# rossng/oxmpl

Measured on AMD Instinct MI355X. Metric: RRT iterations/sec (batched problems), R^3 10k-node tree, 64-sphere field, higher is better.
Workload: dtype f64

## Files before the change

### oxmpl_amd/csrc/oxhip_api.hip

```cpp
#include "../../include/oxmpl_hip.h"

#include <algorithm>
#include <chrono>
#include <cmath>
#include <cstdio>
#include <cstring>
#include <limits>
#include <string>
#include <vector>

#include "oxhip_host.hpp"
#include "oxhip_internal.hpp"
#include "rrt_device.hpp"

using namespace oxhip;

#include <mutex>
#include <utility>
namespace {
std::mutex g_stream_mu;
std::vector<std::pair<int, hipStream_t>> g_stream_pool;
constexpr size_t kStreamPoolMax = 32;
}
namespace oxhip {
// ... 325 lines not shown
    chk(b->goal_r.alloc(P));
    if (!space_of(b).no_body && e == hipSuccess) {
        if (upload(b->se3_body, std::vector<double>(4 * (size_t)kSe3MaxBody, 0.0), b->stream) != OXHIP_OK) e = hipErrorOutOfMemory;
        b->se3.body = b->se3_body.p;
        b->se3.n_body = 1;
    }
    if (e != hipSuccess) return alloc_failed(e);
    dp.tree = b->tree.p; dp.parent = b->parent.p; dp.skip = b->skip.p; dp.state = b->state.p;
    dp.tree_b = b->tree_b.p; dp.parent_b = b->parent_b.p;
    dp.cost = b->cost.p; dp.nb_idx = b->nb_idx.p; dp.nb_dist = b->nb_dist.p;
    dp.wire_chk = b->wire_chk.p; dp.wired = b->wired.p; dp.nbr_cnt = b->nbr_cnt.p; dp.nbr_off = b->nbr_off.p;
    dp.nbr_take = b->nbr_take.p; dp.nbr_total = b->nbr_total.p; dp.d_near = b->d_near.p; dp.pool = b->pool.p;
    dp.chunks = b->chunks.p; dp.chunk_cursor = b->chunk_cursor.p;
    dp.goal_c = b->goal_c.p; dp.goal_thr = b->goal_thr.p; dp.goal_r = b->goal_r.p;
    return OXHIP_OK;
}

static int32_t alloc_cells(oxhip_rrt_batch* b) {
    DevParams& dp = b->dp;
    const uint32_t P = b->cfg.n_problems, dim = b->cfg.dim, cap = dp.cap;
    dp.cell_level_max = cells_level_max(dim, cap);
    dp.cell_blocks = cells_head_blocks(dim, cap) + cap / 7u + 64u;
    uint32_t split = b->cfg.frozen_split;
    if (split == 0) { split = (3072u + P - 1u) / P; if (split > 8u) split = 8u; if (split < 1u) split = 1u; }
    dp.cells_split = split;
    dp.sph_grid_G = sphere_grid_side(dim);
    const size_t grid_cells = dim == 2 ? (size_t)dp.sph_grid_G * dp.sph_grid_G : (size_t)dp.sph_grid_G * dp.sph_grid_G * dp.sph_grid_G;
    size_t off = 0;
    auto carve = [&](size_t bytes) { const size_t at = off; off = (off + bytes + 255u) & ~(size_t)255u; return at; };
    const size_t o_meta = carve((size_t)P * sizeof(CellMeta)), o_acc = carve((size_t)P * sizeof(CellAcc));
    const size_t zero_bytes = off;
    const size_t o_pos = carve((size_t)P * 64 * sizeof(uint64_t)), o_grid = carve(grid_cells * sizeof(uint64_t));
    const size_t o_grid2 = carve(b->star_wired ? grid_cells * sizeof(uint64_t) : 0);
    const size_t o_flat = carve((size_t)P * 4096 * 4 * sizeof(float)), o_xyz = carve((size_t)P * cap * 4 * sizeof(double));
    const size_t o_blk = carve((size_t)P * dp.cell_blocks * sizeof(CellBlock));
    hipError_t e = b->cell_arena.alloc(off);
    if (e == hipSuccess) e = hipMemset(b->cell_arena.p, 0, zero_bytes);
    if (e != hipSuccess) return alloc_failed(e);
    uint8_t* base = b->cell_arena.p;
    b->cell_meta_p = reinterpret_cast<CellMeta*>(base + o_meta);
    b->sph_grid_p = reinterpret_cast<uint64_t*>(base + o_grid);
    if (b->star_wired) b->star_grid_p = reinterpret_cast<uint64_t*>(base + o_grid2);
    dp.cell_blk = reinterpret_cast<CellBlock*>(base + o_blk); dp.cell_flat = reinterpret_cast<float*>(base + o_flat);
    dp.cell_xyz = reinterpret_cast<double*>(base + o_xyz); dp.cell_meta = b->cell_meta_p;
    dp.cell_acc = reinterpret_cast<CellAcc*>(base + o_acc); dp.cell_part_pos = reinterpret_cast<uint64_t*>(base + o_pos);
    dp.sph_grid = b->sph_grid_p;
    return OXHIP_OK;
}

static int32_t alloc_shadow(oxhip_rrt_batch* b) {
    const size_t P = b->cfg.n_problems;
    hipError_t e = b->tree32.alloc(P * b->cfg.dim * b->dp.cap);
    if (e == hipSuccess) e = b->shadow_state.alloc(P * 2);
    if (e == hipSuccess) e = hipMemset(b->shadow_state.p, 0, P * 2 * sizeof(uint32_t));
    if (e != hipSuccess) return alloc_failed(e);
    b->dp.tree32 = b->tree32.p;
    b->dp.shadow_state = b->shadow_state.p;
    return OXHIP_OK;
}

template <typename Launch>
static int32_t op_batch(int32_t device, const double* a, const double* b, const double* t, uint32_t n, double* out,
                        size_t w_a, size_t w_b, size_t w_out, bool b_uploaded, bool t_uploaded, Launch launch) {
    if (n == 0) return OXHIP_OK;
    OX_TRY(select_device(device));
    TmpStream ts;
    OX_TRY(ts.acquire(device));
    DevBuf<double> da, db, dt, dout;
// ... 1012 lines not shown
```

### oxmpl_amd/csrc/rrt_cells.hip

```cpp
#include "oxhip_internal.hpp"
#include "rrt_device.hpp"
#include "rrt_resident_common.hpp"
#include "lane_query_common.hpp"
#include "lane_sampler.hpp"

namespace oxhip {

#ifndef OXHIP_CELLS_BRUTE
#define OXHIP_CELLS_BRUTE 512
#endif
constexpr uint32_t kBruteMax = OXHIP_CELLS_BRUTE;
constexpr uint32_t kFlatCap = 4096;
static_assert(kBruteMax <= kFlatCap, "the flat list holds the small trees");
constexpr int kCellsWaves = 4;
constexpr uint32_t kSelfSkipMax = 4;
constexpr uint32_t kMaxSplit = 64;
constexpr int kMaxShell = 6;
#ifndef OXHIP_CELLS_NB
#define OXHIP_CELLS_NB 4
#endif
#ifndef OXHIP_ABLATE
#define OXHIP_ABLATE 0
#endif
#ifndef OXHIP_CELLS_WT_UNROLL
#define OXHIP_CELLS_WT_UNROLL 4
#endif
#ifndef OXHIP_CELLS_NB_FROZEN
#define OXHIP_CELLS_NB_FROZEN 3
#endif
#ifndef OXHIP_CELLS_FILL_X2
#define OXHIP_CELLS_FILL_X2 7ull
#endif
#ifndef OXHIP_CELLS_TAIL
#define OXHIP_CELLS_TAIL 64
#endif

typedef float cfloat4 __attribute__((ext_vector_type(4)));
typedef uint32_t cuint4 __attribute__((ext_vector_type(4)));
typedef double cdouble4 __attribute__((ext_vector_type(4)));
// ... 21 lines not shown
template <int DIM>
struct CellsShared {
    double obs[DIM + 2][64];
    CellsWaveLds<DIM> w[kCellsWaves];
};

__host__ __device__ __forceinline__ uint32_t cells_G(uint32_t level) {
    const uint32_t t[15] = {1u, 2u, 2u, 3u, 4u, 6u, 8u, 11u, 16u, 23u, 32u, 45u, 64u, 91u, 128u};
    return t[level < 14u ? level : 14u];
}
__host__ __device__ __forceinline__ uint32_t cells_level_cap(uint32_t level, int dim) {
    unsigned long long v = OXHIP_CELLS_FILL_X2;
    for (int k = 0; k < dim; ++k) v *= cells_G(level);
    v >>= 1;
    return v > 0xFFFFFFFEull ? 0xFFFFFFFEu : (uint32_t)v;
}
__device__ __forceinline__ uint32_t cells_level(uint32_t n, int dim, uint32_t level_max) {
    if (n <= kBruteMax) return 0u;
    uint32_t l = 1;
    while (l < level_max && cells_level_cap(l, dim) < n) ++l;
    return l;
}

template <int DIM>
__device__ __forceinline__ void grid_load(const CellMeta& m, CellGrid& g) {
#pragma unroll
    for (int k = 0; k < 3; ++k) {
        g.lo[k] = unid(m.lo[k]);
        g.G[k] = uni(m.G[k]);
    }
    g.inv_h = unid(m.inv_h);
    g.level = uni(m.level);
    g.regrid_at = uni(m.regrid_at);
    g.pool_next = uni(m.pool_next);
    g.delta_node = (double)__builtin_bit_cast(float, uni(__builtin_bit_cast(uint32_t, m.delta_node)));
}

template <int DIM>
__device__ __forceinline__ uint32_t cell_place(const CellGrid& g, const double x[DIM], uint32_t idx, uint64_t& entry, float tf[3], double& err) {
    uint32_t c[3] = {0u, 0u, 0u}, u[3] = {0u, 0u, 0u};
    err = 0.0;
#pragma unroll
    for (int k = 0; k < 3; ++k) {
        tf[k] = 0.0f;
        if (k < DIM) {
            const double t = (x[k] - g.lo[k]) * g.inv_h;
// ... 253 lines not shown
__device__ __forceinline__ double block_lb(const CellGrid& g, const float (&tq)[3], const uint32_t (&cq)[3], uint32_t r) {
    double lb = __builtin_inf();
#pragma unroll
    for (int k = 0; k < DIM; ++k) {
        if (cq[k] > r) lb = fmin(lb, (double)tq[k] - (double)(cq[k] - r));
        if (cq[k] + r + 1u < g.G[k]) lb = fmin(lb, (double)(cq[k] + r + 1u) - (double)tq[k]);
    }
    return lb;
}

__device__ __forceinline__ int cells_verdict(const Top2& t, double lb, double A) {
    if (!(t.s1 < __builtin_inff())) return lb < __builtin_inf() ? 1 : 2;
    const double d1 = sqrt((double)t.s1) * (1.0 + 0x1p-20) + A;
    const double d2 = sqrt((double)t.s2) * (1.0 - 0x1p-20) - A;
    if (!(d1 < d2)) return 2;
    if (!(d1 < lb * (1.0 - 0x1p-20))) return 1;
    return 0;
}

template <int DIM>
__device__ __forceinline__ bool cells_band_resolve(const CellGrid& grid, const CellBlock* blk, const cdouble4* xyz, CellsWaveLds<DIM>* sh, uint32_t lane,
                                                   const double (&q1)[DIM], float s1, double A, uint32_t& idx_out, double& g_out) {
    if (!(s1 < __builtin_inff())) return false;
    float tq[3] = {0.0f, 0.0f, 0.0f};
    uint32_t cq[3] = {0u, 0u, 0u};
#pragma unroll
    for (int k = 0; k < DIM; ++k) {
        tq[k] = (float)((q1[k] - grid.lo[k]) * grid.inv_h);
        const float fl = floorf(tq[k]);
        cq[k] = fl > 0.0f ? (fl < (float)grid.G[k] ? (uint32_t)fl : grid.G[k] - 1u) : 0u;
    }
    const double B = sqrt((double)s1) * (1.0 + 0x1p-20) + 2.0 * A;
    if (!(B < block_lb<DIM>(grid, tq, cq, 1u) * (1.0 - 0x1p-20))) return false;
    const float thr2 = f32_up(B * B * (1.0 + 0x1p-20));
    constexpr uint32_t NC = DIM == 3 ? 27u : 9u;
    const int d[3] = {(int)(lane % 3u) - 1, (int)((lane / 3u) % 3u) - 1, DIM == 3 ? (int)(lane / 9u) - 1 : 0};
    uint32_t cc[3] = {0u, 0u, 0u};
    bool on = lane < NC;
    float gap2 = 0.0f;
#pragma unroll
    for (int k = 0; k < DIM; ++k) {
        const int c = (int)cq[k] + d[k];
        on = on && c >= 0 && c < (int)grid.G[k];
        cc[k] = (uint32_t)c;
        const float gk = (d[k] < 0 ? fmaxf(tq[k] - (float)cq[k], 0.0f) : fmaxf((float)(cq[k] + 1u) - tq[k], 0.0f)) * (1.0f - 0x1p-20f);
        gap2 = d[k] != 0 ? gap2 + gk * gk : gap2;
    }
    on = on && !(gap2 > thr2);
    float off[3];
#pragma unroll
    for (int k = 0; k < 3; ++k) off[k] = ((float)cc[k] + 0x1p-17f) - tq[k];
    cuint4 v[4];
    block_load(blk, on ? (cc[2] * grid.G[1] + cc[1]) * grid.G[0] + cc[0] : 0u, v);
// ... 35 lines not shown
    const float sk = sh->tail_s1[mine ? lane : 0u];
    const cdouble4 c4 = xyz[ik];
    double c[DIM];
#pragma unroll
    for (int k = 0; k < DIM; ++k) c[k] = c4[k];
    const double g = dist2<DIM>(c, q1, DIM);
    Exact e{__builtin_inf(), kNoNode};
    if (mine) { e.dist = sqrt(g); e.idx = ik; }
    e = exact_wave_reduce(e);
    const uint64_t wm = __ballot(mine && ik == e.idx);
    if (wm == 0) return false;
    const int wl = __ffsll((unsigned long long)wm) - 1;
    const double gw = readlane_f64(g, wl);
    const double sw = sqrt((double)lbits_f32((uint32_t)__builtin_amdgcn_readlane((int)lf32_bits(sk), wl)));
    if (!(fabs(sqrt(gw) * grid.inv_h - sw) <= A + sw * 0x1p-19 + 1e-30)) return false;
    idx_out = uni(e.idx);
    g_out = unid(gw);
    return true;
}

#ifndef OXHIP_CELLS_SKIP_COST_INV
#define OXHIP_CELLS_SKIP_COST_INV 16
#endif
__host__ __device__ __forceinline__ uint32_t cells_part_begin(uint32_t rounds, uint32_t part, uint32_t split) {
    if (part >= split) return rounds;
    if (split > kSelfSkipMax) return (uint32_t)(((uint64_t)rounds * part) / split);
    constexpr uint64_t ci = OXHIP_CELLS_SKIP_COST_INV;
    uint64_t full = 1, keep_s = 1, keep_p = 1;
    for (uint32_t i = 0; i < split; ++i) { full *= ci; keep_s *= ci - 1u; keep_p *= i < part ? ci - 1u : ci; }
    return (uint32_t)(((uint64_t)rounds * (full - keep_p)) / (full - keep_s));
}

#ifndef OXHIP_CELLS_WAVES_PER_EU
#define OXHIP_CELLS_WAVES_PER_EU 2
#endif
#ifndef OXHIP_CELLS_WAVES_PER_EU_FROZEN
#define OXHIP_CELLS_WAVES_PER_EU_FROZEN 3
#endif
template <int DIM, bool STAMP, bool FROZEN>
__global__ __launch_bounds__(kCellsWaves * 64, FROZEN ? OXHIP_CELLS_WAVES_PER_EU_FROZEN : OXHIP_CELLS_WAVES_PER_EU) void rrt_cells_kernel(DevParams p) {
    constexpr int D = DIM;
    __shared__ CellsShared<DIM> shared;

    const uint32_t tid = threadIdx.x;
    const uint32_t wave = uni(tid >> 6), lane = tid & 63;
    const uint32_t split = FROZEN ? p.cells_split : 1u;
    const uint32_t xcd = blockIdx.x & 7u, unit = (blockIdx.x >> 3) * (uint32_t)kCellsWaves + wave;
    const uint32_t prob = (unit / split) * 8u + xcd, part = unit % split;

    const uint32_t ns64 = p.n_spheres < 64 ? p.n_spheres : 64;
    const uint32_t nobs = p.n_spheres + p.n_boxes;
    const bool extras = nobs > ns64;
    double c0[D];
#pragma unroll
    for (int k = 0; k < D; ++k) c0[k] = 0.5 * p.lo[k] + 0.5 * p.hi[k];
    if (wave == 0) {
#pragma unroll
        for (int k = 0; k < D; ++k) shared.obs[k][lane] = lane < ns64 ? p.sph_c[(size_t)k * p.n_spheres + lane] : 0.0;
        shared.obs[D][lane] = lane < ns64 ? p.sph_thr[lane] : -1.0;
        shared.obs[D + 1][lane] = lane < ns64 ? p.sph_filt[lane] : -1.0;
    }
    const bool live = prob < p.n_problems;
    const ProblemState st0 = p.state[live ? prob : 0u];
    CellsWaveLds<DIM>* sh = &shared.w[wave];
    CellMeta& meta = p.cell_meta[live ? prob : 0u];
    CellGrid grid;
    grid_load<DIM>(meta, grid);
    LMargins mg;
    {
        double h = (double)lbits_f32(uni(meta.mabs_bits)) * (1.0 + 0x1p-23);
#pragma unroll
        for (int k = 0; k < D; ++k) {
            h = fmax(h, fmax(fabs(p.lo[k] - c0[k]), fabs(p.hi[k] - c0[k])));
            h = fmax(h, fabs(p.goal_c[(size_t)(live ? prob : 0u) * DIM + k] - c0[k]));
        }
        h = unid(h) * 1.001;
        mg.usable = h < 1e15 && fabs(c0[0]) < 1e300;
        mg.e2 = 2.0 * lanes_screen_e(h, D);
    }
    __syncthreads();
    if (!live) return;
    if (p.stop_at_goal && st0.goal_node >= 0) return;
    float sg_inv[D], sg_bias[D];
#pragma unroll
    for (int k = 0; k < D; ++k) {
        const double inv = (double)p.sph_grid_G / (p.hi[k] - p.lo[k]);
        sg_inv[k] = lbits_f32(uni(lf32_bits((float)inv)));
        sg_bias[k] = lbits_f32(uni(lf32_bits((float)((c0[k] - p.lo[k]) * inv))));
    }

    const size_t cap = p.cap;
    double* tree = p.tree + (size_t)prob * DIM * cap;
    int32_t* parent = p.parent + (size_t)prob * cap;
    uint8_t* skip = p.skip + (size_t)prob * cap;
    CellBlock* blk = p.cell_blk + (size_t)prob * p.cell_blocks;
    cfloat4* flat = reinterpret_cast<cfloat4*>(p.cell_flat) + (size_t)prob * kFlatCap;
    cdouble4* xyz = reinterpret_cast<cdouble4*>(p.cell_xyz) + (size_t)prob * cap;
    double goal_c[D];
#pragma unroll
    for (int k = 0; k < D; ++k) goal_c[k] = p.goal_c[(size_t)prob * DIM + k];
    const double goal_thr = p.goal_thr[prob];
    const double goal_radius = p.goal_r[prob];

    const uint32_t budget_all = (uint32_t)p.budget;
    uint32_t j_lo = 0, j_hi = budget_all;
    uint64_t pos_start = st0.draws;
    if (split > 1) {
        const uint32_t rounds = (budget_all + 63u) / 64u;
        j_lo = cells_part_begin(rounds, part, split) * 64u;
        j_hi = cells_part_begin(rounds, part + 1u, split) * 64u;
        if (j_hi > budget_all) j_hi = budget_all;
        if (split > kSelfSkipMax) pos_start = p.cell_part_pos[(size_t)prob * kMaxSplit + part];
    }
    const uint32_t budget = j_hi - j_lo;

    uint64_t pw = 1;
    {
        uint64_t base = kFnvPrime;
#pragma unroll
        for (int b = 0; b < 6; ++b) {
            if ((lane >> b) & 1u) pw *= base;
            base *= base;
        }
    }
    const uint64_t pw64 = uni64(((uint64_t)(uint32_t)__builtin_amdgcn_readlane((int)(uint32_t)(pw >> 32), 63) << 32 |
                                 (uint32_t)__builtin_amdgcn_readlane((int)(uint32_t)pw, 63)) * kFnvPrime);

    RngWindow rng;
    rng.init(sh->rng_buf, p.seed, p.first_problem_id + prob, pos_start);
    if (split > 1 && split <= kSelfSkipMax && j_lo > 0) {
        for (uint32_t r0 = 0; r0 < j_lo; r0 += 64u) cells_sample_block<DIM, false>(rng, p, goal_c, goal_radius, 64u, lane, sh, r0);
        pos_start = rng.pos;
    }
    ProblemState st = st0;
    if (split > 1) { st.checksum = 0; st.accepted = 0; st.iterations = 0; }
    uint64_t draws_done = pos_start;
    uint32_t n = st.n_nodes;
    uint32_t mabs_bits = uni(meta.mabs_bits);
    uint32_t jr = 0, js = 0;
    int32_t stop = 1;
    uint64_t n_rounds = 0, n_lanes = 0, n_amb = 0, n_expand = 0, n_cut_conflict = 0, n_tie = 0, n_memo = 0, n_forced = 0, n_regrid = 0, n_steps = 0, n_tail = 0, n_tail_pairs = 0, n_band = 0;
    uint64_t t_ph[8] = {0, 0, 0, 0, 0, 0, 0, 0}, t_pm = 0, t_c[4] = {0, 0, 0, 0}, t_cm = 0;
    uint64_t h_lanes[8] = {0, 0, 0, 0, 0, 0, 0, 0}, h_cells[8] = {0, 0, 0, 0, 0, 0, 0, 0}, h_trips[8] = {0, 0, 0, 0, 0, 0, 0, 0};
    const uint64_t t_begin = STAMP ? (uint64_t)clock64() : 0;
#define OXHIP_CPHASE(IDX) do { if (STAMP) { const uint64_t now_ = (uint64_t)clock64(); t_ph[IDX] += now_ - t_pm; t_pm = now_; } } while (0)
    uint32_t memo_n = 0xFFFFFFFFu, memo_idx = kNoNode;
    double memo_g = 0.0, memo_q[D];
#pragma unroll
    for (int k = 0; k < D; ++k) memo_q[k] = 0.0;
    typedef double ldouble4 __attribute__((ext_vector_type(4)));

    while (true) {
        if (jr >= budget) { stop = 1; break; }
        if (!FROZEN && n >= p.max_nodes) { stop = 2; break; }
        if (!FROZEN && n >= grid.regrid_at) {
            cells_build<DIM>(p, prob, n, lane, c0, grid, mabs_bits);
            if (STAMP) ++n_regrid;
        }
        uint32_t m = budget - jr < 64u ? budget - jr : 64u;
        if (js < jr + m) {
            cells_sample_block<DIM, true>(rng, p, goal_c, goal_radius, jr + m - js, lane, sh, js);
            js = jr + m;
        }
        if (STAMP) { ++n_rounds; n_lanes += m; t_pm = (uint64_t)clock64(); }
        const bool act = lane < m;
        const uint32_t slot = (jr + (act ? lane : 0u)) & 63u;
        double q[D];
#pragma unroll
        for (int k = 0; k < D; ++k) q[k] = sh->q[k][slot];
        const uint64_t pos_after_l = sh->pos_after[slot];

        Top2 t2{__builtin_inff(), __builtin_inff(), kNoNode};
        float tq[3] = {0.0f, 0.0f, 0.0f};
        uint32_t cq[3] = {0u, 0u, 0u};
#pragma unroll
        for (int k = 0; k < D; ++k) {
            tq[k] = (float)((q[k] - grid.lo[k]) * grid.inv_h);
            const float fl = floorf(tq[k]);
            cq[k] = fl > 0.0f ? (fl < (float)grid.G[k] ? (uint32_t)fl : grid.G[k] - 1u) : 0u;
        }
        const uint32_t gmax = grid.G[0] > grid.G[1] ? (grid.G[0] > grid.G[2] ? grid.G[0] : grid.G[2]) : (grid.G[1] > grid.G[2] ? grid.G[1] : grid.G[2]);
        const double A = sqrt((double)D) * (grid.delta_node + (double)(gmax + 8u) * 0x1p-23) * 1.01 + 1e-30;
        int verdict;
        __builtin_amdgcn_fence(__ATOMIC_RELEASE, "workgroup");
        bool from_memo = act && memo_n == n;
#pragma unroll
        for (int k = 0; k < D; ++k) from_memo = from_memo && __double_as_longlong(q[k]) == __double_as_longlong(memo_q[k]);
        if (grid.level == 0) {
            cfloat4 mine_nd = flat[lane < n ? lane : 0u];
            Top2 ta[4] = {{__builtin_inff(), __builtin_inff(), kNoNode}, {__builtin_inff(), __builtin_inff(), kNoNode},
                          {__builtin_inff(), __builtin_inff(), kNoNode}, {__builtin_inff(), __builtin_inff(), kNoNode}};
            for (uint32_t i0 = 0; i0 < n; i0 += 64) {
                const cfloat4 cur_nd = mine_nd;
                const uint32_t nx = i0 + 64u + lane;
                mine_nd = flat[nx < n ? nx : 0u];
                const uint32_t cnt = n - i0 < 64u ? n - i0 : 64u;
                for (uint32_t t = 0; t < cnt; t += 4) {
#pragma unroll
                    for (int u = 0; u < 4; ++u) {
                        const uint32_t tt = t + (uint32_t)u < cnt ? t + (uint32_t)u : cnt - 1u;
                        cfloat4 nd;
#pragma unroll
// ... 255 lines not shown
            clear = true;
        }
        if (STAMP) n_memo += (uint64_t)__popcll(__ballot(from_memo));
        const bool amb = act && !clear;
        if (FROZEN && __ballot(amb) != 0) sh->tail_s2[lane] = (verdict == 2 && grid.level != 0) ? t2.s1 : __builtin_inff();
        const uint32_t hb = hi32(g) + 1;
        double qn[D], mid[D];
        steer<DIM>(p, false, g, q_near, q, qn);
        bool dup = g == 0.0;
        OXHIP_CPHASE(1);
        float Qf[D];
        double bb = 0.0;
#pragma unroll
        for (int k = 0; k < D; ++k) {
            const float bk = (float)(q[k] - c0[k]);
            Qf[k] = -2.0f * bk;
            bb += (double)bk * (double)bk;
        }
        bool bad = false;
        if (nobs > 0) {
            lerp<DIM>(q_near, qn, 0.5, mid, DIM);
            uint64_t cand;
            {
                const float gs = (float)p.sph_grid_G;
                bool inside = mg.usable && !(OXHIP_ABLATE & 1);
                uint32_t ci[3] = {0u, 0u, 0u};
#pragma unroll
                for (int k = 0; k < D; ++k) {
                    const float u = __builtin_fmaf((float)(mid[k] - c0[k]), sg_inv[k], sg_bias[k]);
                    inside = inside && u >= -0x1p-10f && u <= gs + 0x1p-10f;
                    const float fl = floorf(u);
                    ci[k] = fl > 0.0f ? (fl < gs ? (uint32_t)fl : p.sph_grid_G - 1u) : 0u;
                }
                const uint64_t m = p.sph_grid[D == 3 ? (ci[2] * p.sph_grid_G + ci[1]) * p.sph_grid_G + ci[0] : ci[1] * p.sph_grid_G + ci[0]];
                cand = inside ? m : ~0ull;
            }
            uint32_t maybe_lo = (uint32_t)cand, maybe_hi = (uint32_t)(cand >> 32);
            {
                uint64_t rem = ((uint64_t)maybe_hi << 32) | maybe_lo;
                if (ns64 < 64) rem &= (1ull << ns64) - 1ull;
                uint64_t keep = 0;
                while (__ballot(rem != 0) != 0) {
                    const bool has = rem != 0;
                    const uint32_t o = has ? (uint32_t)(__ffsll((unsigned long long)rem) - 1) : 0u;
                    double c[D];
#pragma unroll
                    for (int k = 0; k < D; ++k) c[k] = shared.obs[k][o];
                    if (has && sphere_maybe_hit<DIM>(c, shared.obs[D + 1][o], mid)) keep |= 1ull << o;
                    rem &= rem - 1;
                }
                maybe_lo = (uint32_t)keep;
                maybe_hi = (uint32_t)(keep >> 32);
            }
// ... 399 lines not shown
                    }
                    if (grid.level != 0) cells_insert(blk, grid.pool_next, cell, entry, lane == 0 && !dup1, lane);
                    if (!dup1 && err > grid.delta_node) grid.delta_node = (double)f32_up(err * (1.0 + 1e-9));
                    {
                        uint32_t mab = 0;
#pragma unroll
                        for (int k = 0; k < D; ++k) { const uint32_t ab = lf32_bits((float)(qn1[k] - c0[k])) & 0x7FFFFFFFu; mab = ab > mab ? ab : mab; }
                        mabs_bits = mab > mabs_bits ? mab : mabs_bits;
                    }
                    ++n;
                    if (dist2<D>(qn1, goal_c, DIM) <= goal_thr) {
                        if (st.goal_node < 0) st.goal_node = (int32_t)i;
                        hit1 = true;
                    }
                }
            }
            if (!FROZEN) jr += 1;
            goal_stop = hit1 && p.stop_at_goal;
        } while (FROZEN && todo != 0);
        if (goal_stop) { stop = 0; break; }
    }
#undef OXHIP_CPHASE
    if (!FROZEN) __builtin_amdgcn_fence(__ATOMIC_RELEASE, "agent");
    if (split > 1) {
        uint64_t w = 1, base = kFnvPrime;
        for (uint32_t e = budget_all - j_hi; e != 0; e >>= 1) { if (e & 1u) w *= base; base *= base; }
        CellAcc& acc = p.cell_acc[prob];
        uint32_t arrived = 0;
        if (lane == 0) {
            const unsigned long long r0 = atomicAdd((unsigned long long*)&acc.chk, (unsigned long long)(st.checksum * w));
            const unsigned long long r1 = atomicAdd((unsigned long long*)&acc.accepted, (unsigned long long)st.accepted);
            const unsigned long long r2 = part == split - 1u ? atomicExch((unsigned long long*)&acc.pos, (unsigned long long)draws_done) : 0ull;
            uint32_t one = 1u;
            asm volatile("" : "+v"(one) : "v"((uint32_t)r0), "v"((uint32_t)r1), "v"((uint32_t)r2));
            arrived = atomicAdd(&acc.done, one);
        }
        arrived = uni(arrived);
        if (arrived == split - 1u && lane == 0) {
            uint64_t pn = 1, b2 = kFnvPrime;
            for (uint32_t e = budget_all; e != 0; e >>= 1) { if (e & 1u) pn *= b2; b2 *= b2; }
            ProblemState out = st0;
            out.checksum = st0.checksum * pn + (uint64_t)atomicAdd((unsigned long long*)&acc.chk, 0ull);
            out.accepted = st0.accepted + (uint64_t)atomicAdd((unsigned long long*)&acc.accepted, 0ull);
            out.iterations = st0.iterations + budget_all;
            out.draws = (uint64_t)atomicAdd((unsigned long long*)&acc.pos, 0ull);
            out.stop_reason = 1;
            p.state[prob] = out;
            acc.chk = 0; acc.accepted = 0; acc.pos = 0; acc.done = 0;
        }
    } else if (lane == 0) {
        st.n_nodes = n;
        st.draws = draws_done;
        st.stop_reason = stop;
        p.state[prob] = st;
    }
    if (!FROZEN) grid_store<DIM>(meta, grid, n, mabs_bits, lane);
    if (STAMP && p.dbg && lane == 0) {
        atomicAdd((unsigned long long*)&p.dbg[54], (unsigned long long)n_amb);
        atomicAdd((unsigned long long*)&p.dbg[55], (unsigned long long)n_memo);
        atomicAdd((unsigned long long*)&p.dbg[56], (unsigned long long)n_cut_conflict);
        atomicAdd((unsigned long long*)&p.dbg[59], (unsigned long long)n_forced);
        atomicAdd((unsigned long long*)&p.dbg[60], (unsigned long long)n_expand);
        atomicAdd((unsigned long long*)&p.dbg[61], (unsigned long long)n_regrid);
        atomicAdd((unsigned long long*)&p.dbg[45], (unsigned long long)n_amb);
        atomicAdd((unsigned long long*)&p.dbg[14], (unsigned long long)n_band);
        {
            const uint64_t life = (uint64_t)clock64() - t_begin;
            atomicAdd((unsigned long long*)&p.dbg[50], (unsigned long long)life);
            atomicMax((unsigned long long*)&p.dbg[51], (unsigned long long)~life);
            atomicMax((unsigned long long*)&p.dbg[52], (unsigned long long)life);
            atomicAdd((unsigned long long*)&p.dbg[53], (unsigned long long)(n_lanes - (st.iterations - (split > 1 ? 0ull : st0.iterations))));
        }
        if (prob == 0) {
            const uint64_t vals[8] = {n_amb, n_rounds, n_lanes, st.iterations, n_expand, n_steps, n_regrid, n_memo};
            const int idx[8] = {4, 5, 6, 7, 8, 9, 10, 11};
            for (int i = 0; i < 8; ++i) atomicAdd((unsigned long long*)&p.dbg[idx[i]], (unsigned long long)vals[i]);
            atomicAdd((unsigned long long*)&p.dbg[12], (unsigned long long)n_cut_conflict);
            atomicAdd((unsigned long long*)&p.dbg[15], (unsigned long long)n_tie);
            for (int i = 0; i < 8; ++i) atomicAdd((unsigned long long*)&p.dbg[32 + i], (unsigned long long)t_ph[i]);
            atomicAdd((unsigned long long*)&p.dbg[13], (unsigned long long)((uint64_t)clock64() - t_begin));
            p.dbg[62] = t_c[0]; p.dbg[63] = t_c[1]; p.dbg[49] = t_c[2]; p.dbg[0] = t_c[3];
            atomicAdd((unsigned long long*)&p.dbg[1], (unsigned long long)n_tail);
            atomicAdd((unsigned long long*)&p.dbg[2], (unsigned long long)n_tail_pairs);
            for (int i = 0; i < 8; ++i) {
                atomicAdd((unsigned long long*)&p.dbg[16 + i], (unsigned long long)h_lanes[i]);
                atomicAdd((unsigned long long*)&p.dbg[24 + i], (unsigned long long)h_trips[i]);
            }
            const int ci[8] = {40, 41, 42, 43, 44, 46, 47, 48};
            for (int i = 0; i < 8; ++i) atomicAdd((unsigned long long*)&p.dbg[ci[i]], (unsigned long long)h_cells[i]);
        }
    }
}

template <int DIM>
__global__ __launch_bounds__(64) void cells_prepare_kernel(DevParams p) {
    __shared__ CellsWaveLds<DIM> shw;
    const uint32_t prob = blockIdx.x, lane = threadIdx.x;
    const ProblemState st0 = p.state[prob];
    if (p.stop_at_goal && st0.goal_node >= 0) return;
    CellMeta& meta = p.cell_meta[prob];
    const uint32_t n = st0.n_nodes;
    double c0[DIM];
#pragma unroll
    for (int k = 0; k < DIM; ++k) c0[k] = 0.5 * p.lo[k] + 0.5 * p.hi[k];
    const bool valid = uni(meta.valid) != 0 && uni(meta.n_grid) == n &&
                       (p.freeze || n < uni(meta.regrid_at)) && uni(meta.level) == cells_level(n, DIM, p.cell_level_max);
    if (!valid) {
        CellGrid g;
        uint32_t mabs_bits;
        cells_build<DIM>(p, prob, n, lane, c0, g, mabs_bits);
        grid_store<DIM>(meta, g, n, mabs_bits, lane);
    }
    const uint32_t split = p.freeze ? p.cells_split : 1u;
    if (split <= kSelfSkipMax) return;
    double goal_c[DIM];
#pragma unroll
    for (int k = 0; k < DIM; ++k) goal_c[k] = p.goal_c[(size_t)prob * DIM + k];
    RngWindow rng;
    rng.init(shw.rng_buf, p.seed, p.first_problem_id + prob, st0.draws);
    const uint32_t budget = (uint32_t)p.budget, rounds = (budget + 63u) / 64u;
    uint32_t next_part = 0;
    for (uint32_t r = 0; r < rounds; ++r) {
        while (next_part < split && cells_part_begin(rounds, next_part, split) == r) {
            if (lane == 0) p.cell_part_pos[(size_t)prob * kMaxSplit + next_part] = rng.pos;
            ++next_part;
        }
        if (next_part >= split) break;
        const uint32_t m = budget - r * 64u < 64u ? budget - r * 64u : 64u;
        cells_sample_block<DIM, false>(rng, p, goal_c, p.goal_r[prob], m, lane, &shw, r * 64u);
    }
    while (next_part < split) {
        if (lane == 0) p.cell_part_pos[(size_t)prob * kMaxSplit + next_part] = rng.pos;
        ++next_part;
    }
}

__global__ __launch_bounds__(256) void sphere_grid_kernel(DevParams p, uint64_t* grid, const double* filt) {
    const uint32_t G = p.sph_grid_G, dim = p.dim;
    const uint32_t cells = dim == 2 ? G * G : G * G * G;
    const uint32_t idx = blockIdx.x * 256u + threadIdx.x;
    if (idx >= cells) return;
    const uint32_t ic[3] = {idx % G, (idx / G) % G, idx / (G * G)};
    const uint32_t ns64 = p.n_spheres < 64 ? p.n_spheres : 64;
    uint64_t mask = 0;
    for (uint32_t j = 0; j < ns64; ++j) {
        double d2 = 0.0;
// ... 8 lines not shown
    }
    grid[idx] = mask;
}
uint32_t sphere_grid_side(uint32_t dim) { return dim == 2 ? 128u : 32u; }
void launch_sphere_grid(const DevParams& p, uint64_t* grid, const double* filt, hipStream_t stream) {
    const uint32_t G = p.sph_grid_G, cells = p.dim == 2 ? G * G : G * G * G;
    hipLaunchKernelGGL(sphere_grid_kernel, dim3((cells + 255u) / 256u), dim3(256), 0, stream, p, grid, filt);
}

bool cells_supported(uint32_t dim, uint32_t cap) { return (dim == 2 || dim == 3) && cap <= 65535u; }

uint32_t cells_level_max(uint32_t dim, uint32_t cap) {
    const uint32_t lim = dim == 2 ? 14u : 10u;
    uint32_t l = 1;
    while (l < lim && cells_level_cap(l, (int)dim) < cap) ++l;
    return l;
}
uint32_t cells_head_blocks(uint32_t dim, uint32_t cap) {
    const uint32_t g = cells_G(cells_level_max(dim, cap));
    return dim == 2 ? g * g : g * g * g;
}

template <int DIM>
static void launch_cells_dim(const DevParams& p, hipStream_t stream) {
    const uint32_t split = p.freeze ? p.cells_split : 1u;
    if (!(p.cells_meta_ok != 0 && split <= kSelfSkipMax))
        hipLaunchKernelGGL((cells_prepare_kernel<DIM>), dim3(p.n_problems), dim3(64), 0, stream, p);
    const uint32_t per_xcd = (p.n_problems + 7u) / 8u;
    const uint32_t wgs_per_xcd = (per_xcd * split + (uint32_t)kCellsWaves - 1u) / (uint32_t)kCellsWaves;
    dim3 grid(8u * wgs_per_xcd), block(kCellsWaves * 64);
    if (p.freeze) {
        if (p.dbg) hipLaunchKernelGGL((rrt_cells_kernel<DIM, true, true>), grid, block, 0, stream, p);
        else hipLaunchKernelGGL((rrt_cells_kernel<DIM, false, true>), grid, block, 0, stream, p);
    } else {
        if (p.dbg) hipLaunchKernelGGL((rrt_cells_kernel<DIM, true, false>), grid, block, 0, stream, p);
        else hipLaunchKernelGGL((rrt_cells_kernel<DIM, false, false>), grid, block, 0, stream, p);
    }
}

void launch_rrt_cells(const DevParams& p, hipStream_t stream) {
    if (p.dim == 2) launch_cells_dim<2>(p, stream);
    else if (p.dim == 3) launch_cells_dim<3>(p, stream);
}

}
```

### oxmpl_amd/csrc/rrt_device.hpp

```cpp
#pragma once

#include <hip/hip_runtime.h>
#include <stdint.h>

#include "../../include/oxmpl_hip.h"
#include "ox_sincos.hpp"

namespace oxhip {

constexpr int kMaxDim = 8;
constexpr uint64_t kFnvPrime = 0x100000001B3ull;
constexpr uint64_t kFnvBasis = 0xCBF29CE484222325ull;

struct ProblemState {
    uint64_t iterations;
    uint64_t accepted;
    uint64_t checksum;
    uint64_t draws;
    uint32_t n_nodes;
    int32_t goal_node;
    int32_t stop_reason;
    uint32_t n_nodes_b;
    int32_t goal_node_b;
    uint32_t pad;
// ... 75 lines not shown
    uint32_t* nbr_off;
    uint32_t* nbr_take;
    uint32_t* nbr_total;
    double* d_near;
    struct StarEntry* pool;
    uint32_t pool_share;
    struct StarChunk* chunks;
    uint32_t* chunk_cursor;
    uint32_t chunk_share;
    uint32_t seg_index, seg_count;
    const double* sph_r;
    double filt_abs;
    float* tree32;
    uint32_t* shadow_state;
    uint32_t dbg_flags;
    uint32_t goal_sampler;
    const double* goal_r;
    CellBlock* cell_blk;
    float* cell_flat;
    double* cell_xyz;
    CellMeta* cell_meta;
    CellAcc* cell_acc;
    uint64_t* cell_part_pos;
    uint32_t cell_blocks, cell_level_max, cells_split;
    uint32_t cells_meta_ok;
    const uint64_t* sph_grid;
    uint32_t sph_grid_G;
    const uint64_t* star_sph_grid;
    double so3_centre[4];
    double so3_max_angle;
};

__device__ __forceinline__ uint32_t uni(uint32_t v) { return __builtin_amdgcn_readfirstlane(v); }
__device__ __forceinline__ uint64_t uni64(uint64_t v) {
    uint32_t lo = __builtin_amdgcn_readfirstlane((uint32_t)v);
    uint32_t hi = __builtin_amdgcn_readfirstlane((uint32_t)(v >> 32));
    return ((uint64_t)hi << 32) | lo;
}
__device__ __forceinline__ double unid(double v) { return __longlong_as_double((long long)uni64((uint64_t)__double_as_longlong(v))); }
__device__ __forceinline__ double readlane_f64(double v, int l) {
    const int lo = __builtin_amdgcn_readlane(__double2loint(v), l), hi = __builtin_amdgcn_readlane(__double2hiint(v), l);
    return __hiloint2double(hi, lo);
}
__device__ __forceinline__ uint64_t below_mask(uint32_t lane) { return (1ull << lane) - 1ull; }

__device__ __forceinline__ uint32_t rotl32(uint32_t v, int c) { return (v << c) | (v >> (32 - c)); }

// ... 455 lines not shown
```

Before: 6.125 billion.

## Add atomic work-claiming of per-problem chunks across XCD queues in cells kernel

In the frozen cells kernel, the fixed assignment of waves to (problem, part) is replaced by a persistent loop. Each wave claims work units from per-XCD atomic head counters and, once its own queue is empty, steals from the other XCDs' queues. The number of parts per problem now follows from the round count (chunks of a few rounds), and the grid is capped at a fixed number of waves. The prepare kernel precomputes RNG positions per part and resets the heads. Several asm pins force values into scalar or vector registers to shape register allocation. This adds atomic traffic, an extra prepare-kernel launch and per-claim setup overhead, in exchange for better load balance when problems take uneven time.

```diff
diff --git a/oxmpl_amd/csrc/oxhip_api.hip b/oxmpl_amd/csrc/oxhip_api.hip
--- a/oxmpl_amd/csrc/oxhip_api.hip
+++ b/oxmpl_amd/csrc/oxhip_api.hip
@@ -371,13 +371,15 @@
     dp.cell_level_max = cells_level_max(dim, cap);
     dp.cell_blocks = cells_head_blocks(dim, cap) + cap / 7u + 64u;
     uint32_t split = b->cfg.frozen_split;
-    if (split == 0) { split = (3072u + P - 1u) / P; if (split > 8u) split = 8u; if (split < 1u) split = 1u; }
+    dp.cells_claim = 0;
+    if (split == 0) { split = (3072u + P - 1u) / P; if (split > 8u) split = 8u; if (split < 1u) split = 1u; dp.cells_claim = split > 1u ? 1u : 0u; }
     dp.cells_split = split;
     dp.sph_grid_G = sphere_grid_side(dim);
     const size_t grid_cells = dim == 2 ? (size_t)dp.sph_grid_G * dp.sph_grid_G : (size_t)dp.sph_grid_G * dp.sph_grid_G * dp.sph_grid_G;
     size_t off = 0;
     auto carve = [&](size_t bytes) { const size_t at = off; off = (off + bytes + 255u) & ~(size_t)255u; return at; };
     const size_t o_meta = carve((size_t)P * sizeof(CellMeta)), o_acc = carve((size_t)P * sizeof(CellAcc));
+    const size_t o_heads = carve(8u * 32u * sizeof(uint32_t));
     const size_t zero_bytes = off;
     const size_t o_pos = carve((size_t)P * 64 * sizeof(uint64_t)), o_grid = carve(grid_cells * sizeof(uint64_t));
     const size_t o_grid2 = carve(b->star_wired ? grid_cells * sizeof(uint64_t) : 0);
@@ -393,6 +395,7 @@
     dp.cell_blk = reinterpret_cast<CellBlock*>(base + o_blk); dp.cell_flat = reinterpret_cast<float*>(base + o_flat);
     dp.cell_xyz = reinterpret_cast<double*>(base + o_xyz); dp.cell_meta = b->cell_meta_p;
     dp.cell_acc = reinterpret_cast<CellAcc*>(base + o_acc); dp.cell_part_pos = reinterpret_cast<uint64_t*>(base + o_pos);
+    dp.cell_heads = reinterpret_cast<uint32_t*>(base + o_heads);
     dp.sph_grid = b->sph_grid_p;
     return OXHIP_OK;
 }
diff --git a/oxmpl_amd/csrc/rrt_cells.hip b/oxmpl_amd/csrc/rrt_cells.hip
--- a/oxmpl_amd/csrc/rrt_cells.hip
+++ b/oxmpl_amd/csrc/rrt_cells.hip
@@ -15,6 +15,11 @@
 constexpr int kCellsWaves = 4;
 constexpr uint32_t kSelfSkipMax = 4;
 constexpr uint32_t kMaxSplit = 64;
+#ifndef OXHIP_CELLS_CHUNK_ROUNDS
+#define OXHIP_CELLS_CHUNK_ROUNDS 2
+#endif
+constexpr uint32_t kClaimWaves = 3072;
+constexpr uint32_t kHeadStride = 32;
 constexpr int kMaxShell = 6;
 #ifndef OXHIP_CELLS_NB
 #define OXHIP_CELLS_NB 4
@@ -82,6 +87,16 @@
     return l;
 }
 
+__device__ __forceinline__ uint32_t pin_u32(uint32_t v) {
+    asm volatile("" : "+v"(v));
+    return __builtin_amdgcn_readfirstlane(v);
+}
+__device__ __forceinline__ float pin_f32(float v) { return lbits_f32(pin_u32(lf32_bits(v))); }
+__device__ __forceinline__ double pin_f64(double v) {
+    const uint64_t b = (uint64_t)__double_as_longlong(v);
+    return __longlong_as_double((long long)(((uint64_t)pin_u32((uint32_t)(b >> 32)) << 32) | pin_u32((uint32_t)b)));
+}
+
 template <int DIM>
 __device__ __forceinline__ void grid_load(const CellMeta& m, CellGrid& g) {
 #pragma unroll
@@ -381,13 +396,16 @@
 __device__ __forceinline__ bool cells_band_resolve(const CellGrid& grid, const CellBlock* blk, const cdouble4* xyz, CellsWaveLds<DIM>* sh, uint32_t lane,
                                                    const double (&q1)[DIM], float s1, double A, uint32_t& idx_out, double& g_out) {
     if (!(s1 < __builtin_inff())) return false;
+    asm volatile("" : "+v"(lane));
     float tq[3] = {0.0f, 0.0f, 0.0f};
     uint32_t cq[3] = {0u, 0u, 0u};
 #pragma unroll
     for (int k = 0; k < DIM; ++k) {
         tq[k] = (float)((q1[k] - grid.lo[k]) * grid.inv_h);
         const float fl = floorf(tq[k]);
-        cq[k] = fl > 0.0f ? (fl < (float)grid.G[k] ? (uint32_t)fl : grid.G[k] - 1u) : 0u;
+        uint32_t gk = grid.G[k];
+        asm volatile("" : "+s"(gk));
+        cq[k] = fl > 0.0f ? (fl < (float)gk ? (uint32_t)fl : gk - 1u) : 0u;
     }
     const double B = sqrt((double)s1) * (1.0 + 0x1p-20) + 2.0 * A;
     if (!(B < block_lb<DIM>(grid, tq, cq, 1u) * (1.0 - 0x1p-20))) return false;
@@ -469,13 +487,18 @@
 #ifndef OXHIP_CELLS_SKIP_COST_INV
 #define OXHIP_CELLS_SKIP_COST_INV 16
 #endif
-__host__ __device__ __forceinline__ uint32_t cells_part_begin(uint32_t rounds, uint32_t part, uint32_t split) {
+__host__ __device__ __forceinline__ uint32_t cells_part_begin(uint32_t rounds, uint32_t part, uint32_t split, bool prepared) {
     if (part >= split) return rounds;
-    if (split > kSelfSkipMax) return (uint32_t)(((uint64_t)rounds * part) / split);
+    if (prepared) return (uint32_t)(((uint64_t)rounds * part) / split);
     constexpr uint64_t ci = OXHIP_CELLS_SKIP_COST_INV;
     uint64_t full = 1, keep_s = 1, keep_p = 1;
     for (uint32_t i = 0; i < split; ++i) { full *= ci; keep_s *= ci - 1u; keep_p *= i < part ? ci - 1u : ci; }
     return (uint32_t)(((uint64_t)rounds * (full - keep_p)) / (full - keep_s));
+}
+
+__host__ __device__ __forceinline__ uint32_t cells_chunks(uint32_t rounds) {
+    const uint32_t c = rounds / (uint32_t)OXHIP_CELLS_CHUNK_ROUNDS;
+    return c > kMaxSplit ? kMaxSplit : (c < 1u ? 1u : c);
 }
 
 #ifndef OXHIP_CELLS_WAVES_PER_EU
@@ -490,53 +513,101 @@
     __shared__ CellsShared<DIM> shared;
 
     const uint32_t tid = threadIdx.x;
-    const uint32_t wave = uni(tid >> 6), lane = tid & 63;
-    const uint32_t split = FROZEN ? p.cells_split : 1u;
-    const uint32_t xcd = blockIdx.x & 7u, unit = (blockIdx.x >> 3) * (uint32_t)kCellsWaves + wave;
-    const uint32_t prob = (unit / split) * 8u + xcd, part = unit % split;
+    const uint32_t wave = uni(tid >> 6), lane0 = tid & 63;
+    uint32_t lane = lane0;
+    uint32_t split = FROZEN ? p.cells_split : 1u;
+    const uint32_t xcd = blockIdx.x & 7u;
+    const bool claim = FROZEN && p.cells_claim != 0;
+    const bool prepared = claim || split > kSelfSkipMax;
+    const bool parts = claim || split > 1u;
 
     const uint32_t ns64 = p.n_spheres < 64 ? p.n_spheres : 64;
     const uint32_t nobs = p.n_spheres + p.n_boxes;
     const bool extras = nobs > ns64;
     double c0[D];
 #pragma unroll
-    for (int k = 0; k < D; ++k) c0[k] = 0.5 * p.lo[k] + 0.5 * p.hi[k];
+    for (int k = 0; k < D; ++k) c0[k] = pin_f64(0.5 * p.lo[k] + 0.5 * p.hi[k]);
     if (wave == 0) {
 #pragma unroll
         for (int k = 0; k < D; ++k) shared.obs[k][lane] = lane < ns64 ? p.sph_c[(size_t)k * p.n_spheres + lane] : 0.0;
         shared.obs[D][lane] = lane < ns64 ? p.sph_thr[lane] : -1.0;
         shared.obs[D + 1][lane] = lane < ns64 ? p.sph_filt[lane] : -1.0;
     }
-    const bool live = prob < p.n_problems;
-    const ProblemState st0 = p.state[live ? prob : 0u];
     CellsWaveLds<DIM>* sh = &shared.w[wave];
-    CellMeta& meta = p.cell_meta[live ? prob : 0u];
+    double h_bounds = 0.0;
+#pragma unroll
+    for (int k = 0; k < D; ++k) h_bounds = fmax(h_bounds, fmax(fabs(p.lo[k] - c0[k]), fabs(p.hi[k] - c0[k])));
+    h_bounds = pin_f64(h_bounds);
+    const bool c0_small = ((uint64_t)__double_as_longlong(c0[0]) & 0x7FFFFFFFFFFFFFFFull) < (uint64_t)__double_as_longlong(1e300);
+    __syncthreads();
+    float sg_inv[D], sg_bias[D];
+#pragma unroll
+    for (int k = 0; k < D; ++k) {
+        const double inv = (double)p.sph_grid_G / (p.hi[k] - p.lo[k]);
+        sg_inv[k] = pin_f32((float)inv);
+        sg_bias[k] = pin_f32((float)((c0[k] - p.lo[k]) * inv));
+    }
+
+    const size_t cap = p.cap;
+    uint32_t budget_all = (uint32_t)p.budget;
+    const uint64_t t_wave = STAMP ? (uint64_t)clock64() : 0;
+    uint64_t n_claims = 0;
+    bool worked = false;
+    uint32_t q_off = 0;
+
+    for (bool first = true;; first = false) {
+    uint32_t prob, part;
+    if (FROZEN) {
+        asm volatile("" : "+v"(lane));
+        asm volatile("" : "+s"(split), "+s"(budget_all));
+    }
+    if (claim) {
+        if (q_off >= 8u) break;
+        const uint32_t qx = (xcd + q_off) & 7u;
+        const uint32_t q_units = qx < p.n_problems ? ((p.n_problems - qx + 7u) >> 3) * split : 0u;
+        uint32_t u = 0, one = 1u;
+        asm volatile("" : "+v"(one));
+        if (q_units != 0 && lane == 0) u = atomicAdd(&p.cell_heads[qx * kHeadStride], one);
+        u = uni(u);
+        if (u >= q_units) { ++q_off; continue; }
+        prob = (u / split) * 8u + qx;
+        part = u % split;
+        if (STAMP) ++n_claims;
+    } else {
+        if (!first) break;
+        const uint32_t unit = (blockIdx.x >> 3) * (uint32_t)kCellsWaves + wave;
+        prob = (unit / split) * 8u + xcd;
+        part = unit % split;
+        if (prob >= p.n_problems) break;
+    }
+    ProblemState st0 = p.state[prob];
+    if (FROZEN) {
+        st0.iterations = uni64(st0.iterations); st0.accepted = uni64(st0.accepted); st0.checksum = uni64(st0.checksum);
+        st0.draws = uni64(st0.draws); st0.n_nodes = uni(st0.n_nodes); st0.goal_node = (int32_t)uni((uint32_t)st0.goal_node);
+        st0.stop_reason = (int32_t)uni((uint32_t)st0.stop_reason); st0.n_nodes_b = uni(st0.n_nodes_b);
+        st0.goal_node_b = (int32_t)uni((uint32_t)st0.goal_node_b); st0.pad = uni(st0.pad);
+    }
+    if (p.stop_at_goal && st0.goal_node >= 0) continue;
+    worked = true;
+    CellMeta& meta = p.cell_meta[prob];
     CellGrid grid;
     grid_load<DIM>(meta, grid);
+    float Gf[3] = {0.0f, 0.0f, 0.0f};
+    if (FROZEN) {
+#pragma unroll
+        for (int k = 0; k < D; ++k) Gf[k] = pin_f32((float)grid.G[k]);
+    }
     LMargins mg;
     {
-        double h = (double)lbits_f32(uni(meta.mabs_bits)) * (1.0 + 0x1p-23);
-#pragma unroll
-        for (int k = 0; k < D; ++k) {
-            h = fmax(h, fmax(fabs(p.lo[k] - c0[k]), fabs(p.hi[k] - c0[k])));
-            h = fmax(h, fabs(p.goal_c[(size_t)(live ? prob : 0u) * DIM + k] - c0[k]));
-        }
-        h = unid(h) * 1.001;
-        mg.usable = h < 1e15 && fabs(c0[0]) < 1e300;
+        double hb = h_bounds;
+        if (FROZEN) asm volatile("" : "+s"(hb));
+        double h = fmax((double)lbits_f32(uni(meta.mabs_bits)) * (1.0 + 0x1p-23), hb);
+#pragma unroll
+        for (int k = 0; k < D; ++k) h = fmax(h, fabs(p.goal_c[(size_t)prob * DIM + k] - c0[k]));
+        h = unid(h) * pin_f64(1.001);
+        mg.usable = h < 1e15 && c0_small;
         mg.e2 = 2.0 * lanes_screen_e(h, D);
     }
-    __syncthreads();
-    if (!live) return;
-    if (p.stop_at_goal && st0.goal_node >= 0) return;
-    float sg_inv[D], sg_bias[D];
-#pragma unroll
-    for (int k = 0; k < D; ++k) {
-        const double inv = (double)p.sph_grid_G / (p.hi[k] - p.lo[k]);
-        sg_inv[k] = lbits_f32(uni(lf32_bits((float)inv)));
-        sg_bias[k] = lbits_f32(uni(lf32_bits((float)((c0[k] - p.lo[k]) * inv))));
-    }
-
-    const size_t cap = p.cap;
     double* tree = p.tree + (size_t)prob * DIM * cap;
     int32_t* parent = p.parent + (size_t)prob * cap;
     uint8_t* skip = p.skip + (size_t)prob * cap;
@@ -545,19 +616,18 @@
     cdouble4* xyz = reinterpret_cast<cdouble4*>(p.cell_xyz) + (size_t)prob * cap;
     double goal_c[D];
 #pragma unroll
-    for (int k = 0; k < D; ++k) goal_c[k] = p.goal_c[(size_t)prob * DIM + k];
-    const double goal_thr = p.goal_thr[prob];
-    const double goal_radius = p.goal_r[prob];
-
-    const uint32_t budget_all = (uint32_t)p.budget;
+    for (int k = 0; k < D; ++k) goal_c[k] = unid(p.goal_c[(size_t)prob * DIM + k]);
+    const double goal_thr = unid(p.goal_thr[prob]);
+    const double goal_radius = unid(p.goal_r[prob]);
+
     uint32_t j_lo = 0, j_hi = budget_all;
     uint64_t pos_start = st0.draws;
-    if (split > 1) {
+    if (parts) {
         const uint32_t rounds = (budget_all + 63u) / 64u;
-        j_lo = cells_part_begin(rounds, part, split) * 64u;
-        j_hi = cells_part_begin(rounds, part + 1u, split) * 64u;
+        j_lo = cells_part_begin(rounds, part, split, prepared) * 64u;
+        j_hi = cells_part_begin(rounds, part + 1u, split, prepared) * 64u;
         if (j_hi > budget_all) j_hi = budget_all;
-        if (split > kSelfSkipMax) pos_start = p.cell_part_pos[(size_t)prob * kMaxSplit + part];
+        if (prepared) pos_start = uni64(p.cell_part_pos[(size_t)prob * kMaxSplit + part]);
     }
     const uint32_t budget = j_hi - j_lo;
 
@@ -575,12 +645,12 @@
 
     RngWindow rng;
     rng.init(sh->rng_buf, p.seed, p.first_problem_id + prob, pos_start);
-    if (split > 1 && split <= kSelfSkipMax && j_lo > 0) {
+    if (split > 1 && !prepared && j_lo > 0) {
         for (uint32_t r0 = 0; r0 < j_lo; r0 += 64u) cells_sample_block<DIM, false>(rng, p, goal_c, goal_radius, 64u, lane, sh, r0);
         pos_start = rng.pos;
     }
     ProblemState st = st0;
-    if (split > 1) { st.checksum = 0; st.accepted = 0; st.iterations = 0; }
+    if (parts) { st.checksum = 0; st.accepted = 0; st.iterations = 0; }
     uint64_t draws_done = pos_start;
     uint32_t n = st.n_nodes;
     uint32_t mabs_bits = uni(meta.mabs_bits);
@@ -593,8 +663,12 @@
 #define OXHIP_CPHASE(IDX) do { if (STAMP) { const uint64_t now_ = (uint64_t)clock64(); t_ph[IDX] += now_ - t_pm; t_pm = now_; } } while (0)
     uint32_t memo_n = 0xFFFFFFFFu, memo_idx = kNoNode;
     double memo_g = 0.0, memo_q[D];
-#pragma unroll
-    for (int k = 0; k < D; ++k) memo_q[k] = 0.0;
+    if (FROZEN) asm("" : "=v"(memo_g));
+#pragma unroll
+    for (int k = 0; k < D; ++k) {
+        memo_q[k] = 0.0;
+        if (FROZEN) asm("" : "=v"(memo_q[k]));
+    }
     typedef double ldouble4 __attribute__((ext_vector_type(4)));
 
     while (true) {
@@ -624,7 +698,7 @@
         for (int k = 0; k < D; ++k) {
             tq[k] = (float)((q[k] - grid.lo[k]) * grid.inv_h);
             const float fl = floorf(tq[k]);
-            cq[k] = fl > 0.0f ? (fl < (float)grid.G[k] ? (uint32_t)fl : grid.G[k] - 1u) : 0u;
+            cq[k] = fl > 0.0f ? (fl < (FROZEN ? Gf[k] : (float)grid.G[k]) ? (uint32_t)fl : grid.G[k] - 1u) : 0u;
         }
         const uint32_t gmax = grid.G[0] > grid.G[1] ? (grid.G[0] > grid.G[2] ? grid.G[0] : grid.G[2]) : (grid.G[1] > grid.G[2] ? grid.G[1] : grid.G[2]);
         const double A = sqrt((double)D) * (grid.delta_node + (double)(gmax + 8u) * 0x1p-23) * 1.01 + 1e-30;
@@ -926,13 +1000,13 @@
             lerp<DIM>(q_near, qn, 0.5, mid, DIM);
             uint64_t cand;
             {
-                const float gs = (float)p.sph_grid_G;
+                const float gs = pin_f32((float)p.sph_grid_G), gs_hi = pin_f32(gs + 0x1p-10f);
                 bool inside = mg.usable && !(OXHIP_ABLATE & 1);
                 uint32_t ci[3] = {0u, 0u, 0u};
 #pragma unroll
                 for (int k = 0; k < D; ++k) {
                     const float u = __builtin_fmaf((float)(mid[k] - c0[k]), sg_inv[k], sg_bias[k]);
-                    inside = inside && u >= -0x1p-10f && u <= gs + 0x1p-10f;
+                    inside = inside && u >= -0x1p-10f && u <= gs_hi;
                     const float fl = floorf(u);
                     ci[k] = fl > 0.0f ? (fl < gs ? (uint32_t)fl : p.sph_grid_G - 1u) : 0u;
                 }
@@ -1378,8 +1452,9 @@
     }
 #undef OXHIP_CPHASE
     if (!FROZEN) __builtin_amdgcn_fence(__ATOMIC_RELEASE, "agent");
-    if (split > 1) {
+    if (parts) {
         uint64_t w = 1, base = kFnvPrime;
+        asm volatile("" : "+v"(w), "+v"(base));
         for (uint32_t e = budget_all - j_hi; e != 0; e >>= 1) { if (e & 1u) w *= base; base *= base; }
         CellAcc& acc = p.cell_acc[prob];
         uint32_t arrived = 0;
@@ -1394,6 +1469,7 @@
         arrived = uni(arrived);
         if (arrived == split - 1u && lane == 0) {
             uint64_t pn = 1, b2 = kFnvPrime;
+            asm volatile("" : "+v"(pn), "+v"(b2));
             for (uint32_t e = budget_all; e != 0; e >>= 1) { if (e & 1u) pn *= b2; b2 *= b2; }
             ProblemState out = st0;
             out.checksum = st0.checksum * pn + (uint64_t)atomicAdd((unsigned long long*)&acc.chk, 0ull);
@@ -1402,7 +1478,9 @@
             out.draws = (uint64_t)atomicAdd((unsigned long long*)&acc.pos, 0ull);
             out.stop_reason = 1;
             p.state[prob] = out;
-            acc.chk = 0; acc.accepted = 0; acc.pos = 0; acc.done = 0;
+            uint64_t zero = 0;
+            asm volatile("" : "+v"(zero));
+            acc.chk = zero; acc.accepted = zero; acc.pos = zero; acc.done = (uint32_t)zero;
         }
     } else if (lane == 0) {
         st.n_nodes = n;
@@ -1420,13 +1498,7 @@
         atomicAdd((unsigned long long*)&p.dbg[61], (unsigned long long)n_regrid);
         atomicAdd((unsigned long long*)&p.dbg[45], (unsigned long long)n_amb);
         atomicAdd((unsigned long long*)&p.dbg[14], (unsigned long long)n_band);
-        {
-            const uint64_t life = (uint64_t)clock64() - t_begin;
-            atomicAdd((unsigned long long*)&p.dbg[50], (unsigned long long)life);
-            atomicMax((unsigned long long*)&p.dbg[51], (unsigned long long)~life);
-            atomicMax((unsigned long long*)&p.dbg[52], (unsigned long long)life);
-            atomicAdd((unsigned long long*)&p.dbg[53], (unsigned long long)(n_lanes - (st.iterations - (split > 1 ? 0ull : st0.iterations))));
-        }
+        atomicAdd((unsigned long long*)&p.dbg[53], (unsigned long long)(n_lanes - (st.iterations - (parts ? 0ull : st0.iterations))));
         if (prob == 0) {
             const uint64_t vals[8] = {n_amb, n_rounds, n_lanes, st.iterations, n_expand, n_steps, n_regrid, n_memo};
             const int idx[8] = {4, 5, 6, 7, 8, 9, 10, 11};
@@ -1446,12 +1518,22 @@
             for (int i = 0; i < 8; ++i) atomicAdd((unsigned long long*)&p.dbg[ci[i]], (unsigned long long)h_cells[i]);
         }
     }
+    }
+    if (STAMP && p.dbg && lane == 0 && worked) {
+        const uint64_t life = (uint64_t)clock64() - t_wave;
+        atomicAdd((unsigned long long*)&p.dbg[50], (unsigned long long)life);
+        atomicMax((unsigned long long*)&p.dbg[51], (unsigned long long)~life);
+        atomicMax((unsigned long long*)&p.dbg[52], (unsigned long long)life);
+        atomicAdd((unsigned long long*)&p.dbg[57], (unsigned long long)n_claims);
+    }
 }
 
 template <int DIM>
 __global__ __launch_bounds__(64) void cells_prepare_kernel(DevParams p) {
     __shared__ CellsWaveLds<DIM> shw;
     const uint32_t prob = blockIdx.x, lane = threadIdx.x;
+    const bool claim = p.freeze && p.cells_claim != 0;
+    if (claim && prob == 0 && lane < 8u) p.cell_heads[lane * kHeadStride] = 0u;
     const ProblemState st0 = p.state[prob];
     if (p.stop_at_goal && st0.goal_node >= 0) return;
     CellMeta& meta = p.cell_meta[prob];
@@ -1468,7 +1550,8 @@
         grid_store<DIM>(meta, g, n, mabs_bits, lane);
     }
     const uint32_t split = p.freeze ? p.cells_split : 1u;
-    if (split <= kSelfSkipMax) return;
+    const bool prepared = claim || split > kSelfSkipMax;
+    if (!prepared) return;
     double goal_c[DIM];
 #pragma unroll
     for (int k = 0; k < DIM; ++k) goal_c[k] = p.goal_c[(size_t)prob * DIM + k];
@@ -1477,7 +1560,7 @@
     const uint32_t budget = (uint32_t)p.budget, rounds = (budget + 63u) / 64u;
     uint32_t next_part = 0;
     for (uint32_t r = 0; r < rounds; ++r) {
-        while (next_part < split && cells_part_begin(rounds, next_part, split) == r) {
+        while (next_part < split && cells_part_begin(rounds, next_part, split, true) == r) {
             if (lane == 0) p.cell_part_pos[(size_t)prob * kMaxSplit + next_part] = rng.pos;
             ++next_part;
         }
@@ -1532,12 +1615,16 @@
 }
 
 template <int DIM>
-static void launch_cells_dim(const DevParams& p, hipStream_t stream) {
+static void launch_cells_dim(const DevParams& p_in, hipStream_t stream) {
+    DevParams p = p_in;
+    const bool claim = p.freeze && p.cells_claim != 0;
+    if (claim) p.cells_split = cells_chunks(((uint32_t)p.budget + 63u) / 64u);
     const uint32_t split = p.freeze ? p.cells_split : 1u;
-    if (!(p.cells_meta_ok != 0 && split <= kSelfSkipMax))
+    if (claim || !(p.cells_meta_ok != 0 && split <= kSelfSkipMax))
         hipLaunchKernelGGL((cells_prepare_kernel<DIM>), dim3(p.n_problems), dim3(64), 0, stream, p);
     const uint32_t per_xcd = (p.n_problems + 7u) / 8u;
-    const uint32_t wgs_per_xcd = (per_xcd * split + (uint32_t)kCellsWaves - 1u) / (uint32_t)kCellsWaves;
+    uint32_t wgs_per_xcd = (per_xcd * split + (uint32_t)kCellsWaves - 1u) / (uint32_t)kCellsWaves;
+    if (claim && wgs_per_xcd > kClaimWaves / (8u * (uint32_t)kCellsWaves)) wgs_per_xcd = kClaimWaves / (8u * (uint32_t)kCellsWaves);
     dim3 grid(8u * wgs_per_xcd), block(kCellsWaves * 64);
     if (p.freeze) {
         if (p.dbg) hipLaunchKernelGGL((rrt_cells_kernel<DIM, true, true>), grid, block, 0, stream, p);
diff --git a/oxmpl_amd/csrc/rrt_device.hpp b/oxmpl_amd/csrc/rrt_device.hpp
--- a/oxmpl_amd/csrc/rrt_device.hpp
+++ b/oxmpl_amd/csrc/rrt_device.hpp
@@ -121,7 +121,9 @@
     CellMeta* cell_meta;
     CellAcc* cell_acc;
     uint64_t* cell_part_pos;
+    uint32_t* cell_heads;
     uint32_t cell_blocks, cell_level_max, cells_split;
+    uint32_t cells_claim;
     uint32_t cells_meta_ok;
     const uint64_t* sph_grid;
     uint32_t sph_grid_G;
```

After: 5.785 billion. -5.6%, worse.
